# Exidekat/TransformerUpscaler

Measured on AMD Instinct MI355X. Metric: images/sec, FastTransformer 2x 720p->1080p inference, higher is better.
Workload: dtype bf16

## Files before the change

### include/tupscale_hip.h

```cpp
#ifndef TUPSCALE_HIP_H
#define TUPSCALE_HIP_H

#ifdef __cplusplus
extern "C" {
#endif

int tup_abi_version(void);

int tup_conv3x3_c3_fwd(const float* x, const void* wp, const float* bias, const float* in_mask,
                       const void* out_mask, void* out, int B, int H, int W, int relu, void* stream);

int tup_conv3x3_c64_fwd(const void* x, const void* wp, const float* bias, const void* add,
                        const void* mask, void* out, int B, int H, int W, int ntiles, int r,
                        int cout_valid, int relu, int out_mode, int in_r, void* stream);

int tup_decoder_fused_fwd(const void* x, const void* w1, const float* b1, const void* wz, const float* b2,
                          float* seamv, float* cseam, float* out, int B, int H, int W, void* stream);

int tup_decoder_fused_parts_fwd(const void* x, const void* w1, const float* b1, const void* wz,
                                float* part, float* seamv, float* cseam, int B, int H, int W, void* stream);

int tup_conv1_compact_fwd(const float* x, void* xc, int B, int H, int W, void* stream);
int tup_conv12_fused_fwd(const void* xc, const void* w1, const float* b1, const void* w2, const float* b2, void* out,
                         int B, int H, int W, void* stream);

int tup_conv5x5_c64_planar_fwd(const void* x, const void* wp, const float* bias, const void* wv,
                               const float* bv, float* out, int B, int H, int W, int r, int relu, void* stream);

int tup_conv3x3_planar_fwd(const float* x, const float* w28, const float* bias, const float* add,
                           float* out, int B, int H, int W, int r, int clamp01, void* stream);

int tup_resize_aa_fwd(const float* in, float* out, const int* ymin, const int* ysize, const float* yw,
                      int KY, const int* xmin, const int* xsize, const float* xw, int KX, int planes,
                      int Hi, int Wi, int Ho, int Wo, int clamp01, void* stream);

int tup_tail_stream_r2_fwd(const float* x, const float* wfu_t, const float* bfu, const float* wfc_t, const float* bfc,
                           const float* ui, float* out, int B, int H, int W, int clamp01, void* stream);

int tup_tail_stream_r2_resize_fwd(const float* x, const float* wfu_t, const float* bfu, const float* wfc_t, const float* bfc,
                                  const float* ui, float* out, const int* ymin, const int* ysize, const float* yw, int KY,
                                  const int* xmin, const int* xsize, const float* xw, int KX, const int* oxb, const int* oyb,
                                  int B, int H, int W, int Ho, int Wo, int sc, int band_h, int ext, int clamp01, void* stream);

int tup_tail_stream_r2_parts_fwd(const float* part, const float* seamv, const float* cseam, const float* b2, int tilesX,
                                 const float* wfu_t, const float* bfu, const float* wfc_t, const float* bfc,
                                 const float* ui, float* out, int B, int H, int W, int clamp01, void* stream);
int tup_tail_stream_r2_resize_parts_fwd(const float* part, const float* seamv, const float* cseam, const float* b2, int tilesX,
                                        const float* wfu_t, const float* bfu, const float* wfc_t, const float* bfc,
                                        const float* ui, float* out, const int* ymin, const int* ysize, const float* yw, int KY,
                                        const int* xmin, const int* xsize, const float* xw, int KX, const int* oxb, const int* oyb,
                                        int B, int H, int W, int Ho, int Wo, int sc, int band_h, int ext, int clamp01, void* stream);

int tup_tail_fused_fwd(const float* x, const float* wfu, const float* bfu, const float* wfc, const float* bfc,
                       const float* ui, float* out, const int* ymin, const int* ysize, const float* yw, int KY,
                       const int* xmin, const int* xsize, const float* xw, int KX, int B, int H, int W, int r,
                       int Ho, int Wo, int EH, int EW, int clamp01, void* stream);

int tup_clamp01_fwd(const float* in, float* out, long long n, void* stream);

int tup_layernorm_fwd(const float* x, const float* gamma, const float* beta, void* y,
                      float* mean, float* rstd, int M, void* stream);

int tup_relpos_bias_expand(const float* table, float* frag, void* stream);

int tup_window_attn_fwd(const void* qkv, const float* bias_frag, void* out, float* lse, int nwin, float drop_p,
                        unsigned int drop_seed, void* stream);

int tup_gemm_tokens_fwd(const void* A, int a_dtype, int lda, const void* Wt, const float* bias,
                        const float* res, const void* aux, void* out, int ldo, int M, int N, int K,
                        int epilogue, float drop_p, unsigned int drop_seed, void* stream);

int tup_ln_gemm_fwd(const float* x, const float* gamma, const float* beta, const void* Wt,
                    const float* bias, void* out, int M, int N, void* stream);

int tup_fused_mlp_fwd(float* x, const float* gamma, const float* beta, const void* w1, const float* b1,
                      const void* w2, const float* b2, int M, void* stream);

int tup_patch_embed_fwd(const void* feat, const void* Wt, const float* bias, float* x_out,
                        int B, int H, int W, void* stream);

int tup_patch_unembed_fwd(const void* x, int x_bf16, const void* Wt, const float* bias, const void* skip,
                          void* out, int B, int H, int W, void* stream);


int tup_rt_patch_embed_fwd(const void* feat, const void* Wt, const float* bias, const float* pos, float* x_out,
                           int B, int H, int W, void* stream);

int tup_rt_patch_unembed_fwd(const float* x, const void* Wt, const float* bias, const void* skip, void* out,
                             int B, int H, int W, void* stream);

int tup_rt_attention_fwd(const void* qkv, void* out, float* lse, int B, int N, float drop_p, unsigned int drop_seed,
                         void* stream);

int tup_rt_attention_bwd(const void* qkv, const void* out, const void* gout, const float* lse, float* work,
                         void* gqkv, int B, int N, float drop_p, unsigned int drop_seed, void* stream);

int tup_layernorm128_fwd(const float* x, const float* gamma, const float* beta, void* y, float* mean, float* rstd,
                         int M, void* stream);

int tup_rt_bicubic_sum_fwd(const float* a, const float* b, float* out, const int* ayi, const float* ayw,
                           const int* axi, const float* axw, const int* byi, const float* byw, const int* bxi,
                           const float* bxw, int planes, int Ha, int Wa, int Hb, int Wb, int Ho, int Wo,
                           int clamp01, void* stream);


int tup_gemm_wgrad(const void* P, int p_dtype, int ldp, const void* Q, int q_dtype, int ldq,
                   float* out, int ldo, int M, int NI, int NJ, void* stream);
int tup_gemm_wgrad_bias(const void* P, int p_dtype, int ldp, const void* Q, int q_dtype, int ldq,
                        float* out, int ldo, float* colsum_out, int M, int NI, int NJ, void* stream);

// ... 172 lines not shown
```

### transformerupscaler_amd/_lib.py

```python
from __future__ import annotations

import ctypes
import os
from ctypes import c_double, c_float, c_int, c_longlong, c_uint, c_void_p

_HERE = os.path.dirname(os.path.abspath(__file__))
LIB_PATH = os.environ.get("TUP_LIB_PATH") or os.path.join(_HERE, "libtupscale_hip.so")
ABI_VERSION = 15

P = c_void_p
I = c_int
F = c_float
U = c_uint

SIGNATURES = {
    "tup_abi_version": [],
    "tup_conv3x3_c3_fwd": [P, P, P, P, P, P, I, I, I, I, P],
    "tup_conv3x3_c64_fwd": [P, P, P, P, P, P, I, I, I, I, I, I, I, I, I, P],
    "tup_conv5x5_c64_planar_fwd": [P, P, P, P, P, P, I, I, I, I, I, P],
    "tup_decoder_fused_fwd": [P, P, P, P, P, P, P, P, I, I, I, P],
    "tup_decoder_fused_parts_fwd": [P, P, P, P, P, P, P, I, I, I, P],
    "tup_conv1_compact_fwd": [P, P, I, I, I, P],
    "tup_conv12_fused_fwd": [P, P, P, P, P, P, I, I, I, P],
    "tup_conv3x3_planar_fwd": [P, P, P, P, P, I, I, I, I, I, P],
    "tup_resize_aa_fwd": [P, P, P, P, P, I, P, P, P, I, I, I, I, I, I, I, P],
    "tup_tail_fused_fwd": [P, P, P, P, P, P, P, P, P, P, I, P, P, P, I, I, I, I, I, I, I, I, I, I, P],
    "tup_tail_stream_r2_fwd": [P, P, P, P, P, P, P, I, I, I, I, P],
    "tup_tail_stream_r2_resize_fwd": [P] * 7 + [P, P, P, I, P, P, P, I, P, P] + [I] * 9 + [P],
    "tup_tail_stream_r2_parts_fwd": [P, P, P, P, I] + [P] * 6 + [I, I, I, I, P],
    "tup_tail_stream_r2_resize_parts_fwd": [P, P, P, P, I] + [P] * 6 + [P, P, P, I, P, P, P, I, P, P] + [I] * 9 + [P],
    "tup_clamp01_fwd": [P, P, c_longlong, P],
    "tup_layernorm_fwd": [P, P, P, P, P, P, I, P],
    "tup_relpos_bias_expand": [P, P, P],
    "tup_window_attn_fwd": [P, P, P, P, I, F, U, P],
    "tup_gemm_tokens_fwd": [P, I, I, P, P, P, P, P, I, I, I, I, I, F, U, P],
    "tup_ln_gemm_fwd": [P, P, P, P, P, P, I, I, P],
    "tup_fused_mlp_fwd": [P, P, P, P, P, P, P, I, P],
    "tup_patch_embed_fwd": [P, P, P, P, I, I, I, P],
    "tup_patch_unembed_fwd": [P, I, P, P, P, P, I, I, I, P],
    "tup_rt_patch_embed_fwd": [P, P, P, P, P, I, I, I, P],
    "tup_rt_patch_unembed_fwd": [P, P, P, P, P, I, I, I, P],
    "tup_rt_attention_fwd": [P, P, P, I, I, F, U, P],
    "tup_rt_attention_bwd": [P, P, P, P, P, P, I, I, F, U, P],
    "tup_layernorm128_fwd": [P, P, P, P, P, P, I, P],
    "tup_layernorm128_bwd": [P, P, P, P, P, P, P, P, P, I, P, F, U, P],
    "tup_rt_patch_wgrad": [P, P, P, I, I, I, P],
    "tup_conv3x3_c64_wgrad_s2d": [P, P, P, P, I, I, I, I, I, P],
    "tup_rt_bicubic_bwd": [P] * 10 + [I, I, I, I, I, P],
    "tup_rt_bicubic_bwd_banded": [P] * 7 + [I, P, P, I, P, P, I, I, I, I, I, P, P],
    "tup_relpos_bias_expand_h": [P, P, I, P],
    "tup_relpos_bias_expand_n_h": [P, P, I, P],
    "tup_window_attn_bwd_h": [P, P, P, P, P, P, P, P, I, I, F, U, P],
    "tup_relpos_bias_reduce_h": [P, P, I, P],
    "tup_wt_patch_wgrad": [P, P, P, I, I, I, I, P],
    "tup_window_attn_fwd_h": [P, P, P, P, I, I, F, U, P],
    "tup_wt_patch_embed_fwd": [P, P, P, P, I, I, I, I, P],
    "tup_wt_patch_unembed_fwd": [P, P, P, P, P, I, I, I, I, P],
    "tup_fused_qkv_attn_fwd": [P, P, P, P, P, P, P, I, P],
    "tup_fused_attn_block_fwd": [P, P, P, P, P, P, P, P, I, P],
    "tup_fused_block_fwd": [P] * 10 + [I, P],
    "tup_fused_blocks32_fwd": [P, P, I, I, P],
    "tup_blocks_stream_fwd": [P, P, P, I, I, P],
    "tup_clock_probe": [P, P],
    "tup_pack_gather": [P, P, I, P, P, c_longlong, I, P],
    "tup_adam_step": [P, P, I, P],
    "tup_grad_accumulate": [P, P, I, P],
    "tup_grad_sumsq_partial": [P, P, I, P, P],
    "tup_grad_guard_finish": [P, I, c_double, I, P, P],
    "tup_adam_step_guarded": [P, P, I, P, P],
    "tup_adam_step_ema": [P, P, I, P, P],
    "tup_patch_pairs": [P, I, I, I, P, P, P, I, P, P, P],
    "tup_l1_loss_partial": [P, P, P, c_longlong, I, P],
    "tup_l1_loss_bwd": [P, P, P, P, c_longlong, P],
    "tup_u8hwc_to_f32chw": [P, P, I, I, I, I, P],
    "tup_f32chw_to_u8hwc": [P, P, I, I, I, I, P],
    "tup_bra_compose": [P, P, P, P, P, P, P, P],
    "tup_bra_backward": [P, P, P, P, P, P, P, P, P, I, I, I, P],
    "tup_bra_chain": [P, P, P, P, P, P, P, P, P, P, P],
    "tup_resize_u8_rows": [P, P, P, P, P, I, I, I, I, I, P],
    "tup_resize_u8_cols": [P, P, P, P, P, P, I, I, I, I, I, I, P],
    "tup_rt_bicubic_sum_fwd": [P, P, P, P, P, P, P, P, P, P, P, I, I, I, I, I, I, I, I, P],
    "tup_quality_f32_partial": [P, P, P, I, I, I, I, F, P],
    "tup_quality_u8hwc_partial": [P, P, P, I, I, I, I, F, P],
    "tup_quality_reduce": [P, P, I, I, I, I, F, P],
    "tup_quality_loss_reduce": [P, P, P, I, I, I, I, I, F, F, F, P],
    "tup_quality_loss_f32_bwd": [P, P, P, P, I, I, I, F, F, F, F, P],
    "tup_gemm_wgrad": [P, I, I, P, I, I, P, I, I, I, I, P],
    "tup_gemm_wgrad_bias": [P, I, I, P, I, I, P, I, P, I, I, I, P],
    "tup_patch_wgrad": [P, P, P, I, I, I, I, P],
    "tup_patch_wgrad_bf16": [P, P, P, I, I, I, I, P],
    "tup_colsum": [P, I, I, P, I, I, P, P],
    "tup_layernorm_bwd": [P, P, P, P, P, P, P, P, P, I, P, F, U, P],
    "tup_relpos_bias_expand_n": [P, P, P],
    "tup_window_attn_bwd": [P, P, P, P, P, P, P, P, I, F, U, P],
    "tup_window_attn_bwd_scratch": [I, I],
    "tup_dropout_bwd": [P, P, c_longlong, F, U, P],
    "tup_relpos_bias_reduce": [P, P, P],
    "tup_patch_unembed_bwd": [P, P, P, I, I, I, P],
    "tup_patch_embed_bwd": [P, P, P, I, I, I, P],
    "tup_patch_embed_bwd_merge": [P, P, P, P, P, P, P, I, I, I, P],
    "tup_conv3x3_c64_wgrad": [P, P, P, P, I, I, I, I, I, P],
    "tup_conv3x3_thin_wgrad": [P, P, P, P, I, I, I, P],
# ... 68 lines not shown
```

### transformerupscaler_amd/csrc/check_resources.py

```python
#!/usr/bin/env python3
import json
import os
import re
import subprocess
import sys

GUARDED = [
    ("fused_attn.hip", ["fused_qkv_attn_kernel"]),
    ("block_stream.hip", ["blocks_stream_kernel"]),
    ("fused_blocks.hip", ["fused_mlp_v2_kernel"]),
    ("conv3x3_c64.hip", ["conv_c64_persistent_kernel", "bra_rows_persistent_kernel", "conv3_thin_rows_kernel"]),
    ("conv_thin.hip", ["conv3x3_c3_persistent_kernel"]),
    ("decoder_fused.hip", ["decoder_fused_kernel"]),
    ("conv12_fused.hip", ["conv12_fused_kernel"]),
    ("gemm_tokens.hip", ["gemm_panel2_kernel", "patch_embed_kernel"]),
    ("conv_bwd.hip", ["conv3x3_wgrad_c64_kernel", "conv3x3_wgrad_thin_kernel", "conv3x3_wgrad_c64_det_kernel", "conv3x3_wgrad_thin_det_kernel"]),
    ("branch_a_train.hip", ["bra_wgrad_kernel"]),
    ("gemm_wgrad.hip", ["gemm_wgrad_wide_kernel"]),
    ("gemm_wgrad.hip", ["gemm_wgrad_kernelILi0ELi0ELb1E", "gemm_wgrad_kernelILi0ELi1ELb1E", "gemm_wgrad_kernelILi1ELi0ELb1E",
                        "gemm_wgrad_kernelILi1ELi1ELb1E", "gemm_wgrad_kernelILi1ELi2ELb1E", "colsum_kernelILb0ELb1E", "colsum_kernelILb1ELb1E"]),
    ("attention_bwd.hip", ["layernorm_bwd_kernelILi2ELb1E", "layernorm_bwd_kernelILi3ELb1E"]),
    ("quality_loss.hip", ["quality_loss_bwd_kernel"]),
    ("grad_accumulate.hip", ["grad_accumulate_kernel"]),
    ("step_guard.hip", ["grad_sumsq_kernel", "guard_finish_kernel", "adam_guarded_kernel"]),
    ("step_guard.hip", ["adam_ema_kernel"]),
    ("patch_pairs.hip", ["patch_pairs_kernel"]),
    ("tail_stream.hip", ["tail_stream_r2_kernel"]),
]
EXEMPT = re.compile(r"fused_qkv_attn_kernel<true, true, true>|fused_qkv_attn_kernelILb1ELb1ELb1E|fused_mlp_v2_kernelILi[1-9]|blocks_stream_kernel<true>|blocks_stream_kernelILb1E")
ALLOWED_BYTES = {"fused_mlp_v2_kernelILi0E": 72}

FIELDS = {
    "sgprs": r"TotalSGPRs: (\d+)", "vgprs": r" VGPRs: (\d+)", "agprs": r"AGPRs: (\d+)",
    "scratch_bytes_per_lane": r"ScratchSize \[bytes/lane\]: (\d+)", "waves_per_simd": r"Occupancy \[waves/SIMD\]: (\d+)",
    "sgpr_spill": r"SGPRs Spill: (\d+)", "vgpr_spill": r"VGPRs Spill: (\d+)",
}


def demangle(names):
    try:
        out = subprocess.run(["c++filt"], input="\n".join(names), capture_output=True, text=True, check=True).stdout.split("\n")
        return dict(zip(names, out))
    except Exception:
        return {n: n for n in names}


def parse(path):
    txt = open(path, errors="replace").read()
    parts = re.split(r"remark: Function Name: (\S+)", txt)
    recs = {}
    for name, body in zip(parts[1::2], parts[2::2]):
        rec = {}
        for k, pat in FIELDS.items():
            m = re.search(pat, body)
            if m:
                rec[k] = int(m.group(1))
        recs[name] = rec
    return recs


def main(argv):
    out_path = None
    files = []
    for a in argv:
        if a.startswith("--out="):
            out_path = a[6:]
        else:
            files.append(a)
    report, bad = {}, []
    for f in sorted(files):
        src = os.path.basename(f).replace(".remarks", ".hip")
        recs = parse(f)
        names = demangle(list(recs))
        for mangled, rec in recs.items():
            nice = names.get(mangled, mangled)
            rec["source"] = src
            guarded = any(src == gsrc and any(fn in mangled for fn in fns) for gsrc, fns in GUARDED) \
                and not (EXEMPT.search(nice) or EXEMPT.search(mangled))
            rec["guarded_no_scratch"] = bool(guarded)
            report[nice] = rec
            cap = max([v for k, v in ALLOWED_BYTES.items() if k in mangled] + [0])
            rec["scratch_cap_bytes_per_lane"] = cap
            if guarded and rec.get("scratch_bytes_per_lane", 0) > cap:
                bad.append((src, nice, rec["scratch_bytes_per_lane"]))
    try:
        hipcc = os.environ.get("HIPCC", "/opt/rocm/bin/hipcc")
        ver = subprocess.run([hipcc, "--version"], capture_output=True, text=True).stdout
        m = re.search(r"HIP version: (\S+)", ver)
        c = re.search(r"clang version (\S+)", ver)
        compiler = {"hip_version": m.group(1) if m else None, "clang_version": c.group(1) if c else None}
    except Exception:
        compiler = {"hip_version": None, "clang_version": None}
    if out_path:
        with open(out_path, "w") as fh:
# ... 14 lines not shown
```

### transformerupscaler_amd/csrc/conv3x3_c64.hip

```cpp
#include "common.h"
#include <stdlib.h>

namespace {

constexpr int TH = 8, TW = 32;
constexpr int in_tile_bytes(int ks) { return (TH + ks - 1) * (TW + ks - 1) * 128; }

enum { OUT_NHWC_BF16 = 0, OUT_PLANAR_F32 = 1 };

template <int CT, int OUT_MODE, int KS>
__global__ __launch_bounds__(256, (CT <= 4 && KS == 3) ? 2 : 1) void conv3x3_c64_kernel(
    const bf16_t* __restrict__ x, const bf16_t* __restrict__ wp, const float* __restrict__ bias,
    const bf16_t* __restrict__ add, const bf16_t* __restrict__ mask,
    void* __restrict__ out, int H, int W, int ntiles, int r, int cout_valid, int relu,
    int tilesX, int tilesY, int in_r)
{
    constexpr int PADK = KS / 2, HALO_W = TW + KS - 1, HALO_H = TH + KS - 1, NPIX_HALO = HALO_H * HALO_W;
    constexpr int NTAPS = KS * KS;
    extern __shared__ __attribute__((aligned(16))) char smem[];
    char* in_lds = smem;
    char* w_lds = smem + in_tile_bytes(KS);
    constexpr int WROWS = CT * 16;
    constexpr int WSLAB = WROWS * 128;
    constexpr int WCH = WROWS * 8;
    constexpr int WREGS = (WCH + 255) / 256;

    const int tid = threadIdx.x, lane = tid & 63, wave = tid >> 6;
    const int g = lane >> 4, p = lane & 15;
    int bid = blockIdx.x;
    const int tx = bid % tilesX; bid /= tilesX;
    const int ty = bid % tilesY;
    const int b = bid / tilesY;
    const int ty0 = ty * TH, tx0 = tx * TW;

    const int nci = in_r * in_r;
    const int Hin = H * in_r, Win = W * in_r;
    const bf16_t* xb = x + (size_t)b * Hin * Win * 64;
    constexpr int NSI = (NPIX_HALO * 8 + 255) / 256;
    auto stage_input = [&](int ci) {
        const int si = ci / in_r, sj = ci - si * in_r;
        u32x4 v[NSI];
        auto pos = [&](int idx, int& q, int& c, size_t& off) -> bool {
            q = idx >> 3; c = idx & 7;
            const int yy = q / HALO_W, xx = q - yy * HALO_W;
            const int iy = ty0 - PADK + yy, ix = tx0 - PADK + xx;
            const bool ok = idx < NPIX_HALO * 8 && iy >= 0 && iy < H && ix >= 0 && ix < W;
            off = ok ? ((size_t)(iy * in_r + si) * Win + (ix * in_r + sj)) * 64 + c * 8 : 0;
            return ok;
        };
#pragma unroll
        for (int k = 0; k < NSI; ++k) {
            int q, c; size_t off;
            pos(tid + k * 256, q, c, off);
            v[k] = *reinterpret_cast<const u32x4*>(xb + off);
        }
#pragma unroll
        for (int k = 0; k < NSI; ++k) {
            const int idx = tid + k * 256;
            int q, c; size_t off;
            const bool ok = pos(idx, q, c, off);
            if (idx < NPIX_HALO * 8) *reinterpret_cast<u32x4*>(in_lds + swz128(q, c)) = ok ? v[k] : u32x4{0u, 0u, 0u, 0u};
        }
    };
    stage_input(0);

    u32x4 wreg[WREGS];
    auto wload = [&](int it) {
#pragma unroll
        for (int u = 0; u < WREGS; ++u) {
            const int idx = tid + u * 256;
            if (idx < WCH) wreg[u] = *reinterpret_cast<const u32x4*>(wp + (size_t)it * WROWS * 64 + idx * 8);
        }
    };
    auto wstore = [&](int buf) {
#pragma unroll
        for (int u = 0; u < WREGS; ++u) {
            const int idx = tid + u * 256;
            if (idx < WCH) *reinterpret_cast<u32x4*>(w_lds + buf * WSLAB + swz128(idx >> 3, idx & 7)) = wreg[u];
        }
    };

    int qb[4];
#pragma unroll
// ... 736 lines not shown
    }
    const float bv = (bias && g < cout) ? bias[g] : 0.f;
    const uint32_t pbase = lds_addr(smem) + (uint32_t)(2 * wave * T3_HW * 128) + (uint32_t)swz128(p, g);

    f32x4 acc[2][2];
    auto compute_tile = [&]() {
        bf16x8 pf[6][4];
#pragma unroll
        for (int st = 0; st < 6; ++st)
#pragma unroll
            for (int i = 0; i < 4; ++i) {
                const int off = ((i >> 1) + (st >> 1)) * (T3_HW * 128) + (i & 1) * 2048;
                pf[st][i] = (st & 1) ? lds_read_b128_asm_off_x64(pbase, off) : lds_read_b128_asm_off(pbase, off);
            }
#pragma unroll
        for (int i = 0; i < 4; ++i) acc[i >> 1][i & 1] = f32x4{0.f, 0.f, 0.f, 0.f};
#pragma unroll
        for (int st = 0; st < 6; ++st) {
            if (st == 0) lds_wait<15>(); else if (st == 1) lds_wait<15>(); else if (st == 2) lds_wait<12>();
            else if (st == 3) lds_wait<8>(); else if (st == 4) lds_wait<4>(); else lds_wait<0>();
            __builtin_amdgcn_sched_barrier(0);
#pragma unroll
            for (int i = 0; i < 4; ++i) acc[i >> 1][i & 1] = mfma16x16x32(wfr[st >> 1][st & 1], pf[st][i], acc[i >> 1][i & 1]);
            __builtin_amdgcn_sched_barrier(0);
        }
    };
#define TUP_ADD_DPP(a, v, ctrl) asm("v_add_f32_dpp %0, %1, %0 " ctrl " row_mask:0xf bank_mask:0xf bound_ctrl:1" : "+v"(a) : "v"(v))
    auto store_tile = [&](int tile) {
        int t = tile;
        const int tx = t % tilesX; t /= tilesX;
        const int ty = t % tilesY;
        const int b = t / tilesY;
        float* outb = out + ((size_t)b * cout + g) * H * W;
#pragma unroll
        for (int rw = 0; rw < 2; ++rw) {
            const int oy = ty * TH + 2 * wave + rw;
#pragma unroll
            for (int cg = 0; cg < 2; ++cg) {
                const int xo = cg * 16 + p, ox = tx * T3_TW + xo;
                float v = acc[rw][cg][0] + bv;
                TUP_ADD_DPP(v, acc[rw][cg][1], "row_shl:1"); TUP_ADD_DPP(v, acc[rw][cg][2], "row_shl:2");
                if (cg == 0) { TUP_ADD_DPP(v, acc[rw][1][1], "row_shr:15"); TUP_ADD_DPP(v, acc[rw][1][2], "row_shr:14"); }
                if (relu) v = fmaxf(v, 0.f);
                if (g < cout && oy < H && ox < W && xo < T3_TW) outb[(size_t)oy * W + ox] = v;
            }
        }
    };
#undef TUP_ADD_DPP

    int first, stride, limit;
    if ((gridDim.x & 7) == 0) {
        const int per = gridDim.x >> 3, band = (total_tiles + 7) >> 3, start = (blockIdx.x & 7) * band;
        limit = min(total_tiles, start + band);
        first = start + (blockIdx.x >> 3);
        stride = per;
    } else {
        limit = total_tiles; first = blockIdx.x; stride = gridDim.x;
    }
    if (first < limit) prefetch_tile(first);
    for (int tile = first; tile < limit; tile += stride) {
        asm volatile("s_waitcnt vmcnt(0)" ::: "memory");
        __builtin_amdgcn_s_barrier();
        compute_tile();
        asm volatile("s_waitcnt lgkmcnt(0)" ::: "memory");
        __builtin_amdgcn_s_barrier();
        if (tile + stride < limit) prefetch_tile(tile + stride);
        store_tile(tile);
    }
}

int launch_thin_rows(const void* x, const void* wp, const float* bias, float* out, int B, int H, int W, int cout, int relu, hipStream_t s)
{
    const int tilesX = (W + T3_TW - 1) / T3_TW, tilesY = (H + TH - 1) / TH;
    const long long nt = (long long)tilesX * tilesY * B;
    if (nt > 0x7fffffffLL) return (int)hipErrorInvalidValue;
    const int grid = (int)(nt < 768 ? nt : 768);
    conv3_thin_rows_kernel<<<dim3(grid), dim3(256), T3_IN_BYTES, s>>>((const bf16_t*)x, (const bf16_t*)wp, bias, out, B, H, W, cout, relu, tilesX, tilesY);
    TUP_CHECK_LAUNCH();
    return 0;
}

__global__ __launch_bounds__(256) void conv5x5_border_fix_kernel(
    const bf16_t* __restrict__ x, const bf16_t* __restrict__ wv, const float* __restrict__ bv,
    float* __restrict__ out, int B, int H, int W, int r, int relu)
{
    const int lane = threadIdx.x & 63;
    const int Hs = H * r, Ws = W * r, rr = r * r, nout = 3 * rr;
    const int per_img = 2 * Ws + 2 * (Hs - 2);
    const long long gid = (long long)blockIdx.x * 4 + (threadIdx.x >> 6);
    if (gid >= (long long)per_img * B) return;
    const int b = (int)(gid / per_img);
    int k = (int)(gid - (long long)b * per_img);
    int Y, X;
    if (k < Ws) { Y = 0; X = k; }
    else if (k < 2 * Ws) { Y = Hs - 1; X = k - Ws; }
    else { k -= 2 * Ws; Y = 1 + (k >> 1); X = (k & 1) ? Ws - 1 : 0; }
    const int rowmode = (Y == 0) ? 1 : (Y == Hs - 1 ? 2 : 0), colmode = (X == 0) ? 1 : (X == Ws - 1 ? 2 : 0);
    const int v = rowmode * 3 + colmode;
    const int y = Y / r, si = Y - y * r, xx0 = X / r, sj = X - xx0 * r;
    const int sp = si * r + sj;
    float a0 = 0.f, a1 = 0.f, a2 = 0.f;
    const int t8 = lane >> 3, c8 = lane & 7;
    u32x4 fx[4], fw[4][3];
    bool use[4];
#pragma unroll
    for (int rd = 0; rd < 4; ++rd) {
        const int tap = rd * 8 + t8;
        const int ty = tap / 5, tx = tap - ty * 5;
        const int iy = y + ty - 2, ix = xx0 + tx - 2;
        use[rd] = tap < 25 && iy >= 0 && iy < H && ix >= 0 && ix < W;
        const int tapc = tap < 25 ? tap : 24, iyc = min(max(iy, 0), H - 1), ixc = min(max(ix, 0), W - 1);
        fx[rd] = *reinterpret_cast<const u32x4*>(x + (((size_t)b * H + iyc) * W + ixc) * 64 + c8 * 8);
        const bf16_t* wb = wv + (((size_t)v * nout) * 25 + tapc) * 64 + c8 * 8;
#pragma unroll
        for (int c = 0; c < 3; ++c) fw[rd][c] = *reinterpret_cast<const u32x4*>(wb + (size_t)(c * rr + sp) * 25 * 64);
    }
#pragma unroll
    for (int rd = 0; rd < 4; ++rd) {
        if (!use[rd]) continue;
#pragma unroll
        for (int q = 0; q < 4; ++q) {
            const float xl = __builtin_bit_cast(float, fx[rd][q] << 16), xh = __builtin_bit_cast(float, fx[rd][q] & 0xffff0000u);
            a0 = fmaf(xl, __builtin_bit_cast(float, fw[rd][0][q] << 16), a0); a0 = fmaf(xh, __builtin_bit_cast(float, fw[rd][0][q] & 0xffff0000u), a0);
            a1 = fmaf(xl, __builtin_bit_cast(float, fw[rd][1][q] << 16), a1); a1 = fmaf(xh, __builtin_bit_cast(float, fw[rd][1][q] & 0xffff0000u), a1);
            a2 = fmaf(xl, __builtin_bit_cast(float, fw[rd][2][q] << 16), a2); a2 = fmaf(xh, __builtin_bit_cast(float, fw[rd][2][q] & 0xffff0000u), a2);
        }
    }
#pragma unroll
    for (int o = 32; o >= 1; o >>= 1) { a0 += __shfl_xor(a0, o); a1 += __shfl_xor(a1, o); a2 += __shfl_xor(a2, o); }
    if (lane < 3) {
        float val = (lane == 0 ? a0 : (lane == 1 ? a1 : a2)) + bv[v * nout + lane * rr + sp];
        if (relu) val = fmaxf(val, 0.f);
        out[(((size_t)b * 3 + lane) * Hs + Y) * Ws + X] = val;
    }
}

}

extern "C" int tup_conv3x3_c64_fwd(const void* x, const void* wp, const float* bias, const void* add,
                                   const void* mask, void* out, int B, int H, int W, int ntiles, int r,
                                   int cout_valid, int relu, int out_mode, int in_r, void* stream)
{
    if (B <= 0 || H <= 0 || W <= 0) return 0;
    if (in_r < 1 || in_r > 6) return (int)hipErrorInvalidValue;
    const int tilesX = (W + TW - 1) / TW, tilesY = (H + TH - 1) / TH;
    const long long nblk = (long long)tilesX * tilesY * B;
    if (nblk > 0x7fffffffLL) return (int)hipErrorInvalidValue;
    hipStream_t s = reinterpret_cast<hipStream_t>(stream);
    static const bool use_persistent = !TUP_ENV_FLAG("TUP_CONV_NONPERSISTENT");
    if (in_r == 1 && use_persistent) {
        if (out_mode == OUT_NHWC_BF16) {
            if (ntiles != r * r || r < 1) return (int)hipErrorInvalidValue;
            return launch_persistent<4, OUT_NHWC_BF16, 3>(x, wp, bias, add, mask, out, B, H, W, ntiles, r, 64, relu, s);
        }
        if (out_mode == OUT_PLANAR_F32) {
            if (ntiles != 1 || r != 1 || cout_valid < 1 || cout_valid > 16 || add || mask) return (int)hipErrorInvalidValue;
            static const bool thin_pingpong = TUP_ENV_FLAG("TUP_THIN_PINGPONG");
            if (cout_valid <= 4 && !thin_pingpong) return launch_thin_rows(x, wp, bias, (float*)out, B, H, W, cout_valid, relu, s);
            return launch_persistent<1, OUT_PLANAR_F32, 3>(x, wp, bias, nullptr, nullptr, out, B, H, W, 1, 1, cout_valid, relu, s);
        }
        return (int)hipErrorInvalidValue;
    }
    if (out_mode == OUT_NHWC_BF16) {
        if (ntiles != r * r || r < 1) return (int)hipErrorInvalidValue;
        const size_t lds = in_tile_bytes(3) + 2 * 64 * 128;
        conv3x3_c64_kernel<4, OUT_NHWC_BF16, 3><<<dim3((unsigned)nblk), dim3(256), lds, s>>>(
            (const bf16_t*)x, (const bf16_t*)wp, bias, (const bf16_t*)add, (const bf16_t*)mask, out, H, W, ntiles, r,
            64, relu, tilesX, tilesY, in_r);
    } else if (out_mode == OUT_PLANAR_F32) {
        if (ntiles != 1 || r != 1 || cout_valid < 1 || cout_valid > 16 || add || mask) return (int)hipErrorInvalidValue;
        const size_t lds = in_tile_bytes(3) + 2 * 16 * 128;
        conv3x3_c64_kernel<1, OUT_PLANAR_F32, 3><<<dim3((unsigned)nblk), dim3(256), lds, s>>>(
            (const bf16_t*)x, (const bf16_t*)wp, bias, nullptr, nullptr, out, H, W, 1, 1, cout_valid, relu, tilesX,
            tilesY, in_r);
    } else {
        return (int)hipErrorInvalidValue;
    }
    TUP_CHECK_LAUNCH();
    return 0;
}

extern "C" int tup_conv5x5_c64_planar_fwd(const void* x, const void* wp, const float* bias, const void* wv,
                                          const float* bv, float* out, int B, int H, int W, int r, int relu,
                                          void* stream)
{
    if (B <= 0 || H <= 0 || W <= 0) return 0;
    if (!(r == 2 || r == 3 || r == 6)) return (int)hipErrorInvalidValue;
    const int tilesX = (W + TW - 1) / TW, tilesY = (H + TH - 1) / TH;
    const long long nblk = (long long)tilesX * tilesY * B;
    if (nblk > 0x7fffffffLL) return (int)hipErrorInvalidValue;
    hipStream_t s = reinterpret_cast<hipStream_t>(stream);
    const int nout = 3 * r * r;
    static const bool use_persistent5 = !TUP_ENV_FLAG("TUP_CONV_NONPERSISTENT");
    static const bool use_taps25 = TUP_ENV_FLAG("TUP_BRA_TAPS25");
    if (r == 2 && use_persistent5) {
        int e = use_taps25 ? launch_persistent<1, OUT_PLANAR_F32, 5>(x, wp, bias, nullptr, nullptr, out, B, H, W, 1, r, nout, relu, s)
                           : launch_bra_rows(x, wp, bias, out, B, H, W, relu, s);
        if (e) return e;
    } else if (r == 2) {
        conv3x3_c64_kernel<1, OUT_PLANAR_F32, 5><<<dim3((unsigned)nblk), dim3(256), in_tile_bytes(5) + 2 * 16 * 128, s>>>(
            (const bf16_t*)x, (const bf16_t*)wp, bias, nullptr, nullptr, out, H, W, 1, r, nout, relu, tilesX, tilesY, 1);
    } else if (r == 3) {
        const size_t lds = in_tile_bytes(5) + 2 * 32 * 128;
        TUP_SET_DYN_LDS((conv3x3_c64_kernel<2, OUT_PLANAR_F32, 5>), lds);
        conv3x3_c64_kernel<2, OUT_PLANAR_F32, 5><<<dim3((unsigned)nblk), dim3(256), lds, s>>>(
            (const bf16_t*)x, (const bf16_t*)wp, bias, nullptr, nullptr, out, H, W, 1, r, nout, relu, tilesX, tilesY, 1);
    } else {
        const size_t lds = in_tile_bytes(5) + 2 * 112 * 128;
        TUP_SET_DYN_LDS((conv3x3_c64_kernel<7, OUT_PLANAR_F32, 5>), lds);
        conv3x3_c64_kernel<7, OUT_PLANAR_F32, 5><<<dim3((unsigned)nblk), dim3(256), lds, s>>>(
            (const bf16_t*)x, (const bf16_t*)wp, bias, nullptr, nullptr, out, H, W, 1, r, nout, relu, tilesX, tilesY, 1);
    }
    TUP_CHECK_LAUNCH();
    const long long nborder = (long long)B * (2LL * W * r + 2LL * (H * r - 2));
    conv5x5_border_fix_kernel<<<dim3((unsigned)((nborder + 3) / 4)), dim3(256), 0, s>>>(
        (const bf16_t*)x, (const bf16_t*)wv, bv, out, B, H, W, r, relu);
    TUP_CHECK_LAUNCH();
    return 0;
}

#ifdef TUP_DIAG
extern "C" int tup_debug_conv_stamps(unsigned long long* host_out)
{
    return (int)hipMemcpyFromSymbol(host_out, HIP_SYMBOL(tup_conv_stamps), sizeof(unsigned long long) * 2 * 16 * 5);
}
#endif
```

### transformerupscaler_amd/ops.py

```python
from __future__ import annotations

import contextlib
import ctypes
import struct

import numpy as np
import torch

from . import _lib, resize_taps

BF16, F16, F32 = torch.bfloat16, torch.float16, torch.float32
_DTYPE_CODE = {BF16: 0, F32: 1}


_raw_stream = getattr(torch._C, "_cuda_getCurrentRawStream", None)
_cur_dev = torch.cuda.current_device


def _stream():
    if _raw_stream is not None:
        return _raw_stream(_cur_dev())
    return torch.cuda.current_stream().cuda_stream


# ... 75 lines not shown
    return torch.zeros(shape, dtype=F32, device=device)


def conv1(x, wp, bias, relu=True, in_mask=None, out_mask=None):
    B, C, H, W = x.shape
    assert C == 3
    out = torch.empty((B, H, W, 64), dtype=BF16, device=x.device)
    _lib.call("tup_conv3x3_c3_fwd", _chk(x, F32, None, "x"), _chk(wp, BF16, (64, 32), "wp"),
              _opt(bias, F32, (64,), "bias"), _opt(in_mask, F32, x.shape, "in_mask"),
              _opt(out_mask, BF16, out.shape, "out_mask"), out.data_ptr(), B, H, W, int(relu), _stream())
    return out


def conv1_compact(x):
    B, C, H, W = x.shape
    assert C == 3
    xc = torch.empty((B, (H + 7) // 8 * 8 + 4, (W + 31) // 32 * 32 + 4, 4), dtype=BF16, device=x.device)
    _lib.call("tup_conv1_compact_fwd", _chk(x, F32, None, "x"), xc.data_ptr(), B, H, W, _stream())
    return xc


def conv12_fused(xc, H, W, w1, b1, w2, b2):
    B = xc.shape[0]
    _chk(xc, BF16, (B, (H + 7) // 8 * 8 + 4, (W + 31) // 32 * 32 + 4, 4), "xc")
    out = torch.empty((B, H, W, 64), dtype=BF16, device=xc.device)
    _lib.call("tup_conv12_fused_fwd", xc.data_ptr(), _chk(w1, BF16, (64, 32), "w1"), _chk(b1, F32, (64,), "b1"),
              _chk(w2, BF16, (1, 1, 9, 64, 64), "w2"), _chk(b2, F32, (1, 64), "b2"), out.data_ptr(), B, H, W, _stream())
    return out


def conv_c64(x, wp, bias, r=1, relu=False, add=None, mask=None, in_r=1, out=None):
    B, Hi, Wi, C = x.shape
    assert C == 64 and Hi % in_r == 0 and Wi % in_r == 0
    H, W = Hi // in_r, Wi // in_r
    nt = r * r
    if out is None:
        out = torch.empty((B, H * r, W * r, 64), dtype=BF16, device=x.device)
    else:
        _chk(out, BF16, (B, H * r, W * r, 64), "out")
    _lib.call("tup_conv3x3_c64_fwd", _chk(x, BF16, None, "x"), _chk(wp, BF16, (nt, in_r * in_r, 9, 64, 64), "wp"),
              _opt(bias, F32, (nt, 64), "bias"), _opt(add, BF16, out.shape, "add"), _opt(mask, BF16, out.shape, "mask"),
              out.data_ptr(), B, H, W, nt, r, 64, int(relu), 0, in_r, _stream())
    return out


def conv_c64_thin(x, wp, bias, cout, relu=False, out=None):
    B, H, W, C = x.shape
    assert C == 64 and 1 <= cout <= 16
    if out is None:
        out = torch.empty((B, cout, H, W), dtype=F32, device=x.device)
    else:
        _chk(out, F32, (B, cout, H, W), "out")
    _lib.call("tup_conv3x3_c64_fwd", _chk(x, BF16, None, "x"), _chk(wp, BF16, (1, 1, 9, 16, 64), "wp"),
              _opt(bias, F32, (cout,), "bias"), None, None, out.data_ptr(), B, H, W, 1, 1, cout, int(relu), 1, 1, _stream())
    return out


def decoder_fused(x, w1, b1, wz, b2, finish=True):
    B, H, W, C = x.shape
    assert C == 64
    out = torch.empty((B, 3, H, W), dtype=F32, device=x.device)
    seamv = torch.empty((B, 3, H, W), dtype=F32, device=x.device)
    cseam = torch.empty((B, H, (W + 31) // 32, 32), dtype=F32, device=x.device)
    if not finish:
        _chk(b2, F32, (3,), "b2")
        _lib.call("tup_decoder_fused_parts_fwd", _chk(x, BF16, None, "x"), _chk(w1, BF16, (1, 1, 9, 64, 64), "w1"),
                  _chk(b1, F32, (1, 64), "b1"), _chk(wz, BF16, (48, 64), "wz"), out.data_ptr(), seamv.data_ptr(), cseam.data_ptr(),
                  B, H, W, _stream())
        return out, seamv, cseam, b2
    _lib.call("tup_decoder_fused_fwd", _chk(x, BF16, None, "x"), _chk(w1, BF16, (1, 1, 9, 64, 64), "w1"), _chk(b1, F32, (1, 64), "b1"),
              _chk(wz, BF16, (48, 64), "wz"), _chk(b2, F32, (3,), "b2"), seamv.data_ptr(), cseam.data_ptr(), out.data_ptr(),
              B, H, W, _stream())
    return out


def branch_a_composed(x, wp, bias, wv, bv, r, relu=True):
    B, H, W, C = x.shape
    assert C == 64 and r in (2, 3, 6)
    rows, n = {2: 16, 3: 32, 6: 112}[r], 3 * r * r
    out = torch.empty((B, 3, H * r, W * r), dtype=F32, device=x.device)
    _lib.call("tup_conv5x5_c64_planar_fwd", _chk(x, BF16, None, "x"), _chk(wp, BF16, (1, 1, 25, rows, 64), "wp"),
              _chk(bias, F32, (n,), "bias"), _chk(wv, BF16, (9, n, 25, 64), "wv"), _chk(bv, F32, (9, n), "bv"),
              out.data_ptr(), B, H, W, r, int(relu), _stream())
    return out


def conv_planar(x, w28, bias, r=1, add=None, clamp=False):
    B, C, H, W = x.shape
    assert C == 3
    cout = 3 * r * r
    both = clamp == "both"
    shape = (B, 3, H * r, W * r)
    out = torch.empty(((2,) if both else ()) + shape, dtype=F32, device=x.device)
    _lib.call("tup_conv3x3_planar_fwd", _chk(x, F32, None, "x"), _chk(w28, F32, (cout, 28), "w28"),
              _opt(bias, F32, (cout,), "bias"), _opt(add, F32, shape, "add"), out.data_ptr(),
              B, H, W, r, 2 if both else int(bool(clamp)), _stream())
    return (out[0], out[1]) if both else out


def resize_aa(x, size, clamp=False):
    B, C, Hi, Wi = x.shape
    Ho, Wo = size
    ylo, yn, yw, ky = _taps_on(x.device, Hi, Ho)
    xlo, xn, xw, kx = _taps_on(x.device, Wi, Wo)
    both = clamp == "both"
    out = torch.empty(((2,) if both else ()) + (B, C, Ho, Wo), dtype=F32, device=x.device)
    _lib.call("tup_resize_aa_fwd", _chk(x, F32, None, "x"), out.data_ptr(), ylo.data_ptr(), yn.data_ptr(),
              yw.data_ptr(), ky, xlo.data_ptr(), xn.data_ptr(), xw.data_ptr(), kx, B * C, Hi, Wi, Ho, Wo,
              2 if both else int(bool(clamp)), _stream())
    return (out[0], out[1]) if both else out


TAIL_TILE_H = 16


def tail_fused(x, wfu, bfu, wfc, bfc, ui, r, out_hw, clamp=True):
    B, C, H, W = x.shape
    Hs, Ws = H * r, W * r
    Ho, Wo = out_hw
    ylo, yn, yw, ky, xlo, xn, xw, kx, eh, ew = _table(resize_taps.tail_fused_tables, x.device, (Hs, Ws, Ho, Wo, TAIL_TILE_H, 64))
    out = torch.empty((B, 3, Ho, Wo), dtype=F32, device=x.device)
    _lib.call("tup_tail_fused_fwd", _chk(x, F32, None, "x"), _chk(wfu, F32, (3 * r * r, 28), "wfu"), _chk(bfu, F32, (3 * r * r,), "bfu"),
              _chk(wfc, F32, (3, 28), "wfc"), _chk(bfc, F32, (3,), "bfc"), _chk(ui, F32, (B, 3, Hs, Ws), "ui"), out.data_ptr(),
              ylo.data_ptr(), yn.data_ptr(), yw.data_ptr(), ky, xlo.data_ptr(), xn.data_ptr(), xw.data_ptr(), kx,
              B, H, W, r, Ho, Wo, eh, ew, int(clamp), _stream())
    return out


TAIL_STREAM_WAVES_PER_SIMD = 3


def _tail_stream_plan(device, B, H, W, Ho, Wo):
    return _table(resize_taps.tail_stream_plan, device, (B, H, W, Ho, Wo, 256 * 4 * TAIL_STREAM_WAVES_PER_SIMD))


def tail_stream_fits(B, H, W, out_hw=None):
    if B * 12 * H * W >= 1 << 29:
        return False
    if out_hw is not None and tuple(out_hw) != (2 * H, 2 * W) and B * 3 * int(out_hw[0]) * int(out_hw[1]) >= 1 << 29:
        return False
    return True


def tail_stream_r2(x, wfu_t, bfu, wfc_t, bfc, ui, clamp=True, out_hw=None, parts=None):
    if parts is not None:
        part, seamv, cseam, b2 = parts
        B, C, H, W = part.shape
        dev, tiles_x = part.device, (W + 31) // 32
        head = (_chk(part, F32, (B, 3, H, W), "part"), _chk(seamv, F32, (B, 3, H, W), "seamv"),
                _chk(cseam, F32, (B, H, tiles_x, 32), "cseam"), _chk(b2, F32, (3,), "b2"), tiles_x)
        suffix = "_parts_fwd"
    else:
        B, C, H, W = x.shape
        dev = x.device
        head = (_chk(x, F32, (B, 3, H, W), "x"),)
        suffix = "_fwd"
    args = head + (_chk(wfu_t, F32, (27, 12), "wfu_t"), _chk(bfu, F32, (12,), "bfu"),
                   _chk(wfc_t, F32, (27, 4), "wfc_t"), _chk(bfc, F32, (3,), "bfc"), _chk(ui, F32, (B, 3, 2 * H, 2 * W), "ui"))
    if out_hw is None or tuple(out_hw) == (2 * H, 2 * W):
        out = torch.empty((B, 3, 2 * H, 2 * W), dtype=F32, device=dev)
        _lib.call("tup_tail_stream_r2" + suffix, *args, out.data_ptr(), B, H, W, int(clamp), _stream())
        return out
    Ho, Wo = int(out_hw[0]), int(out_hw[1])
    plan = _tail_stream_plan(dev, B, H, W, Ho, Wo)
    if plan is None:
        return None
# ... 846 lines not shown
```

Before: 2631.

## Compute branch-A border pixels with MFMA kernel over 16-pixel edge groups

Replaces the per-pixel wave border-fix kernel for the 5x5 composed branch with an MFMA kernel. Each wave handles 16 border input pixels along one edge and computes all output rows via 16x16x32 bf16 MFMA, double-buffering the row fragments. A small corner-only pass fixes the four corner pixels. The aim is to cut the cost of the border pass, which ran one wave per output border pixel with scalar dot products. It adds kernel complexity and register pressure, and the old path stays available behind an env flag.

After: 2654 (median of 6 runs). About the same (+0.9%).

```diff
diff --git a/include/tupscale_hip.h b/include/tupscale_hip.h
--- a/include/tupscale_hip.h
+++ b/include/tupscale_hip.h
@@ -26,6 +26,8 @@
 
 int tup_conv5x5_c64_planar_fwd(const void* x, const void* wp, const float* bias, const void* wv,
                                const float* bv, float* out, int B, int H, int W, int r, int relu, void* stream);
+int tup_bra_border_fwd(const void* x, const void* wv, const float* bv, float* out, int B, int H, int W, int r, int relu,
+                       int form, void* stream);
 
 int tup_conv3x3_planar_fwd(const float* x, const float* w28, const float* bias, const float* add,
                            float* out, int B, int H, int W, int r, int clamp01, void* stream);
diff --git a/transformerupscaler_amd/_lib.py b/transformerupscaler_amd/_lib.py
--- a/transformerupscaler_amd/_lib.py
+++ b/transformerupscaler_amd/_lib.py
@@ -18,6 +18,7 @@
     "tup_conv3x3_c3_fwd": [P, P, P, P, P, P, I, I, I, I, P],
     "tup_conv3x3_c64_fwd": [P, P, P, P, P, P, I, I, I, I, I, I, I, I, I, P],
     "tup_conv5x5_c64_planar_fwd": [P, P, P, P, P, P, I, I, I, I, I, P],
+    "tup_bra_border_fwd": [P, P, P, P, I, I, I, I, I, I, P],
     "tup_decoder_fused_fwd": [P, P, P, P, P, P, P, P, I, I, I, P],
     "tup_decoder_fused_parts_fwd": [P, P, P, P, P, P, P, I, I, I, P],
     "tup_conv1_compact_fwd": [P, P, I, I, I, P],
diff --git a/transformerupscaler_amd/csrc/check_resources.py b/transformerupscaler_amd/csrc/check_resources.py
--- a/transformerupscaler_amd/csrc/check_resources.py
+++ b/transformerupscaler_amd/csrc/check_resources.py
@@ -10,6 +10,7 @@
     ("block_stream.hip", ["blocks_stream_kernel"]),
     ("fused_blocks.hip", ["fused_mlp_v2_kernel"]),
     ("conv3x3_c64.hip", ["conv_c64_persistent_kernel", "bra_rows_persistent_kernel", "conv3_thin_rows_kernel"]),
+    ("conv3x3_c64.hip", ["bra_border_mfma_kernel"]),
     ("conv_thin.hip", ["conv3x3_c3_persistent_kernel"]),
     ("decoder_fused.hip", ["decoder_fused_kernel"]),
     ("conv12_fused.hip", ["conv12_fused_kernel"]),
diff --git a/transformerupscaler_amd/csrc/conv3x3_c64.hip b/transformerupscaler_amd/csrc/conv3x3_c64.hip
--- a/transformerupscaler_amd/csrc/conv3x3_c64.hip
+++ b/transformerupscaler_amd/csrc/conv3x3_c64.hip
@@ -1,4 +1,5 @@
 #include "common.h"
+#include <type_traits>
 #include <stdlib.h>
 
 namespace {
@@ -901,17 +902,18 @@
 
 __global__ __launch_bounds__(256) void conv5x5_border_fix_kernel(
     const bf16_t* __restrict__ x, const bf16_t* __restrict__ wv, const float* __restrict__ bv,
-    float* __restrict__ out, int B, int H, int W, int r, int relu)
+    float* __restrict__ out, int B, int H, int W, int r, int relu, int corners)
 {
     const int lane = threadIdx.x & 63;
     const int Hs = H * r, Ws = W * r, rr = r * r, nout = 3 * rr;
-    const int per_img = 2 * Ws + 2 * (Hs - 2);
+    const int per_img = corners ? 4 : 2 * Ws + 2 * (Hs - 2);
     const long long gid = (long long)blockIdx.x * 4 + (threadIdx.x >> 6);
     if (gid >= (long long)per_img * B) return;
     const int b = (int)(gid / per_img);
     int k = (int)(gid - (long long)b * per_img);
     int Y, X;
-    if (k < Ws) { Y = 0; X = k; }
+    if (corners) { Y = (k >> 1) ? Hs - 1 : 0; X = (k & 1) ? Ws - 1 : 0; }
+    else if (k < Ws) { Y = 0; X = k; }
     else if (k < 2 * Ws) { Y = Hs - 1; X = k - Ws; }
     else { k -= 2 * Ws; Y = 1 + (k >> 1); X = (k & 1) ? Ws - 1 : 0; }
     const int rowmode = (Y == 0) ? 1 : (Y == Hs - 1 ? 2 : 0), colmode = (X == 0) ? 1 : (X == Ws - 1 ? 2 : 0);
@@ -952,6 +954,139 @@
         if (relu) val = fmaxf(val, 0.f);
         out[(((size_t)b * 3 + lane) * Hs + Y) * Ws + X] = val;
     }
+}
+
+template <int NT> struct BorderFrags { bf16x8 a[NT][10], b[10]; };
+
+template <int NT>
+__global__ __launch_bounds__(256) void bra_border_mfma_kernel(
+    const bf16_t* __restrict__ x, const bf16_t* __restrict__ wv, const float* __restrict__ bv,
+    float* __restrict__ out, int B, int H, int W, int r, int relu)
+{
+    const int lane = threadIdx.x & 63, g = lane >> 4, p = lane & 15;
+    const int wave = __builtin_amdgcn_readfirstlane((int)(threadIdx.x >> 6));
+    const int Hs = H * r, Ws = W * r, rr = r * r, nout = 3 * rr, nrow = 3 * r;
+    const int gw = (W + 15) >> 4, gh = (H + 15) >> 4, per_img = 2 * (gw + gh);
+    const long long task = (long long)blockIdx.x * 4 + wave;
+    if (task >= (long long)per_img * B) return;
+    const int b = (int)(task / per_img);
+    int k = (int)(task - (long long)b * per_img);
+    const bool rowside = k < 2 * gw;
+    if (!rowside) k -= 2 * gw;
+    const int ng = rowside ? gw : gh;
+    const bool last = k >= ng;
+    const int grp = last ? k - ng : k;
+    const int fix = last ? (rowside ? H : W) - 1 : 0;
+    const int sfix = last ? r - 1 : 0;
+    const int v = (last ? 2 : 1) * (rowside ? 3 : 1);
+    const int q = grp * 16 + p;
+    const int py = rowside ? fix : q, px = rowside ? q : fix;
+    const int ty_lo = rowside ? max(0, 2 - fix) : 0, ty_hi = rowside ? min(4, H + 1 - fix) : 4;
+    auto row_of = [&](int j, int& c) { c = j / r; const int s = j - c * r; return c * rr + (rowside ? sfix * r + s : s * r + sfix); };
+
+    const bf16_t* wa[NT];
+#pragma unroll
+    for (int nt = 0; nt < NT; ++nt) {
+        int c;
+        const int n = row_of(min(nt * 16 + p, nrow - 1), c);
+        wa[nt] = wv + ((size_t)(v * nout + n) * 25) * 64 + g * 8;
+    }
+    const bf16_t* xb = x + (size_t)b * H * W * 64 + g * 8;
+
+    auto load_row = [&](BorderFrags<NT>& f, int ty) {
+        const int iyc = min(max(py + ty - 2, 0), H - 1);
+#pragma unroll
+        for (int tx = 0; tx < 5; ++tx) {
+            const int ixc = min(max(px + tx - 2, 0), W - 1);
+            const bf16_t* src = xb + ((size_t)iyc * W + ixc) * 64;
+#pragma unroll
+            for (int half = 0; half < 2; ++half) {
+                f.b[tx * 2 + half] = *reinterpret_cast<const bf16x8*>(src + half * 32);
+#pragma unroll
+                for (int nt = 0; nt < NT; ++nt)
+                    f.a[nt][tx * 2 + half] = *reinterpret_cast<const bf16x8*>(wa[nt] + (ty * 5 + tx) * 64 + half * 32);
+            }
+        }
+    };
+    f32x4 acc[NT][5];
+#pragma unroll
+    for (int nt = 0; nt < NT; ++nt)
+#pragma unroll
+        for (int i = 0; i < 5; ++i) acc[nt][i] = f32x4{0.f, 0.f, 0.f, 0.f};
+    auto mul_row = [&](const BorderFrags<NT>& f, int ty) {
+        const int iy = py + ty - 2;
+        const bool oky = iy >= 0 && iy < H;
+#pragma unroll
+        for (int tx = 0; tx < 5; ++tx) {
+            const int ix = px + tx - 2;
+            const bool ok = oky && ix >= 0 && ix < W;
+#pragma unroll
+            for (int half = 0; half < 2; ++half) {
+                const u32x4 raw = __builtin_bit_cast(u32x4, f.b[tx * 2 + half]);
+                const bf16x8 bb = __builtin_bit_cast(bf16x8, ok ? raw : u32x4{0u, 0u, 0u, 0u});
+#pragma unroll
+                for (int nt = 0; nt < NT; ++nt) acc[nt][tx] = mfma16x16x32(f.a[nt][tx * 2 + half], bb, acc[nt][tx]);
+            }
+        }
+    };
+
+    BorderFrags<NT> f[2];
+    auto run = [&](auto nrows_c) {
+        constexpr int N = decltype(nrows_c)::value;
+        load_row(f[0], ty_lo);
+        if (N > 1) load_row(f[1], ty_lo + 1);
+#pragma unroll
+        for (int i = 0; i < N; ++i) {
+            mul_row(f[i & 1], ty_lo + i);
+            if (i + 2 < N) load_row(f[i & 1], ty_lo + i + 2);
+        }
+    };
+    const int nrows = ty_hi - ty_lo + 1;
+    if (nrows == 5) run(std::integral_constant<int, 5>{});
+    else if (nrows == 3) run(std::integral_constant<int, 3>{});
+    else if (nrows == 2) run(std::integral_constant<int, 2>{});
+    else run(std::integral_constant<int, 1>{});
+
+    if (q >= (rowside ? W : H)) return;
+#pragma unroll
+    for (int nt = 0; nt < NT; ++nt) {
+        const f32x4 sum = ((acc[nt][0] + acc[nt][4]) + acc[nt][2]) + (acc[nt][1] + acc[nt][3]);
+#pragma unroll
+        for (int e = 0; e < 4; ++e) {
+            const int j = nt * 16 + 4 * g + e;
+            if (j >= nrow) continue;
+            int c;
+            const int n = row_of(j, c), s = j - c * r;
+            const int Y = rowside ? fix * r + sfix : q * r + s, X = rowside ? q * r + s : fix * r + sfix;
+            if ((Y == 0 || Y == Hs - 1) && (X == 0 || X == Ws - 1)) continue;
+            float val = sum[e] + bv[v * nout + n];
+            if (relu) val = fmaxf(val, 0.f);
+            out[(((size_t)b * 3 + c) * Hs + Y) * Ws + X] = val;
+        }
+    }
+}
+
+int launch_bra_border(const void* x, const void* wv, const float* bv, float* out, int B, int H, int W, int r, int relu, int form,
+                      hipStream_t s)
+{
+    const bf16_t* xp = (const bf16_t*)x;
+    const bf16_t* wvp = (const bf16_t*)wv;
+    if (form == 0) {
+        const long long nborder = (long long)B * (2LL * W * r + 2LL * (H * r - 2));
+        conv5x5_border_fix_kernel<<<dim3((unsigned)((nborder + 3) / 4)), dim3(256), 0, s>>>(xp, wvp, bv, out, B, H, W, r, relu, 0);
+        TUP_CHECK_LAUNCH();
+        return 0;
+    }
+    const long long ntask = (long long)B * 2 * ((W + 15) / 16 + (H + 15) / 16);
+    const dim3 grid((unsigned)((ntask + 3) / 4));
+    if (r == 6) bra_border_mfma_kernel<2><<<grid, dim3(256), 0, s>>>(xp, wvp, bv, out, B, H, W, r, relu);
+    else        bra_border_mfma_kernel<1><<<grid, dim3(256), 0, s>>>(xp, wvp, bv, out, B, H, W, r, relu);
+    TUP_CHECK_LAUNCH();
+    if (form == 1) {
+        conv5x5_border_fix_kernel<<<dim3((unsigned)B), dim3(256), 0, s>>>(xp, wvp, bv, out, B, H, W, r, relu, 1);
+        TUP_CHECK_LAUNCH();
+    }
+    return 0;
 }
 
 }
@@ -1031,11 +1166,16 @@
             (const bf16_t*)x, (const bf16_t*)wp, bias, nullptr, nullptr, out, H, W, 1, r, nout, relu, tilesX, tilesY, 1);
     }
     TUP_CHECK_LAUNCH();
-    const long long nborder = (long long)B * (2LL * W * r + 2LL * (H * r - 2));
-    conv5x5_border_fix_kernel<<<dim3((unsigned)((nborder + 3) / 4)), dim3(256), 0, s>>>(
-        (const bf16_t*)x, (const bf16_t*)wv, bv, out, B, H, W, r, relu);
-    TUP_CHECK_LAUNCH();
-    return 0;
+    static const bool border_wave = TUP_ENV_FLAG("TUP_BRA_BORDER_WAVE");
+    return launch_bra_border(x, wv, bv, out, B, H, W, r, relu, border_wave ? 0 : 1, s);
+}
+
+extern "C" int tup_bra_border_fwd(const void* x, const void* wv, const float* bv, float* out, int B, int H, int W, int r,
+                                  int relu, int form, void* stream)
+{
+    if (B <= 0 || H <= 0 || W <= 0) return 0;
+    if (!(r == 2 || r == 3 || r == 6) || form < 0 || form > 2) return (int)hipErrorInvalidValue;
+    return launch_bra_border(x, wv, bv, out, B, H, W, r, relu, form, reinterpret_cast<hipStream_t>(stream));
 }
 
 #ifdef TUP_DIAG
diff --git a/transformerupscaler_amd/ops.py b/transformerupscaler_amd/ops.py
--- a/transformerupscaler_amd/ops.py
+++ b/transformerupscaler_amd/ops.py
@@ -181,6 +181,15 @@
     _lib.call("tup_conv5x5_c64_planar_fwd", _chk(x, BF16, None, "x"), _chk(wp, BF16, (1, 1, 25, rows, 64), "wp"),
               _chk(bias, F32, (n,), "bias"), _chk(wv, BF16, (9, n, 25, 64), "wv"), _chk(bv, F32, (9, n), "bv"),
               out.data_ptr(), B, H, W, r, int(relu), _stream())
+    return out
+
+
+def bra_border(x, wv, bv, r, out, relu=True, form=1):
+    B, H, W, C = x.shape
+    assert C == 64 and r in (2, 3, 6) and form in (0, 1, 2)
+    n = 3 * r * r
+    _lib.call("tup_bra_border_fwd", _chk(x, BF16, None, "x"), _chk(wv, BF16, (9, n, 25, 64), "wv"), _chk(bv, F32, (9, n), "bv"),
+              _chk(out, F32, (B, 3, H * r, W * r), "out"), B, H, W, r, int(relu), form, _stream())
     return out
 
 
```
